# fmfi-compbio/nadavca

Hardware: NVIDIA B200
Metric: signal_samples_aligned_per_sec (higher is better)
Workload: dtype f64

## Files before the change

include/nadavca_b200.h:

```cpp
#ifndef NADAVCA_B200_H
#define NADAVCA_B200_H

#include <stdint.h>

#ifdef __cplusplus
extern "C" {
#endif

#define NVB_OK 0
#define NVB_EINVAL (-1)
#define NVB_ECUDA (-2)
#define NVB_ENOMEM (-3)
#define NVB_ESTATE (-4)

#define NVB_READ_OK 0
#define NVB_READ_NO_PATH 1
#define NVB_READ_BAD_BAND 2

typedef struct nvb_model nvb_model;
typedef struct nvb_batch nvb_batch;

int nvb_abi_version(void);
const char *nvb_last_error(void);
int nvb_device_count(void);
int nvb_trim_memory(int device);
#define NVB_SWEEP_AUTO 0
#define NVB_SWEEP_ROTATE 1
#define NVB_SWEEP_STRIPES 2
int nvb_set_sweep_schedule(int schedule);

nvb_model *nvb_model_create(int k, int central_position, int alphabet_size, const double *mean,
                            const double *sigma, int64_t n_kmers, int device);
void nvb_model_destroy(nvb_model *model);
int nvb_model_k(const nvb_model *model);
int nvb_model_central_position(const nvb_model *model);
int nvb_model_alphabet_size(const nvb_model *model);
int nvb_model_expected_signal(nvb_model *model, int32_t n_reads, const int32_t *reference,
                              const int64_t *reference_off, const int32_t *context_before,
                              const int64_t *context_before_off, const int32_t *context_after,
                              const int64_t *context_after_off, double *out);

typedef struct nvb_reads {
  int32_t n_reads;
  const double *signal;
  const int64_t *signal_off;
  const int32_t *reference;
  const int64_t *reference_off;
  const int32_t *context_before;
  const int64_t *context_before_off;
  const int32_t *context_after;
  const int64_t *context_after_off;
  const int32_t *anchors;
  const int64_t *anchor_off;
  int32_t bandwidth;
  int32_t min_event_length;
} nvb_reads;


int nvb_refine_alignment_batch(nvb_model *model, const nvb_reads *reads, int model_transitions, int32_t *events,
                               int32_t *status);
int nvb_estimate_log_likelihoods_batch(nvb_model *model, const nvb_reads *reads, int model_wobbling, double *out,
                                       int32_t *status);

nvb_batch *nvb_batch_create(nvb_model *model, const nvb_reads *reads);
void nvb_batch_destroy(nvb_batch *batch);
int nvb_batch_set_signal(nvb_batch *batch, const double *signal);
int nvb_batch_set_workspace_limit(nvb_batch *batch, int64_t bytes);
int nvb_batch_refine(nvb_batch *batch, int model_transitions, void *stream);
int nvb_batch_estimate(nvb_batch *batch, int model_wobbling, void *stream);
int nvb_batch_get_events(nvb_batch *batch, int32_t *events, int32_t *status);
int nvb_batch_get_log_likelihoods(nvb_batch *batch, double *out, int32_t *status);
int nvb_batch_get_bands(nvb_batch *batch, int32_t *starts, int32_t *ends);
int nvb_batch_cell_counts(nvb_batch *batch, int model_wobbling, int64_t counts[4]);
double *nvb_batch_d_log_likelihoods(nvb_batch *batch);
int32_t *nvb_batch_d_events(nvb_batch *batch);
int32_t *nvb_batch_d_status(nvb_batch *batch);
int nvb_batch_debug_rows(nvb_batch *batch, int read, int plane, double *out_log, int64_t n_cells);
int64_t nvb_batch_launch_count(const nvb_batch *batch);
#define NVB_N_STAGES 4
int nvb_batch_enable_timing(nvb_batch *batch, int on);
int nvb_batch_get_timing(nvb_batch *batch, double ms[NVB_N_STAGES], int64_t launches[NVB_N_STAGES]);
int nvb_measure_fp64_fma_rate(int device, double *fma_per_second);
// ... 50 lines not shown
```

nadavca_b200/_cabi.py:

```python
import ctypes
import os

import numpy as np

_HERE = os.path.dirname(os.path.abspath(__file__))
LIB_PATH = os.path.join(_HERE, 'libnadavca_b200.so')

NVB_READ_OK, NVB_READ_NO_PATH, NVB_READ_BAD_BAND = 0, 1, 2


class NadavcaCudaError(RuntimeError):
    pass


c_i32p = ctypes.POINTER(ctypes.c_int32)
c_i64p = ctypes.POINTER(ctypes.c_int64)
c_f64p = ctypes.POINTER(ctypes.c_double)
c_i8p = ctypes.POINTER(ctypes.c_int8)


class NvbReads(ctypes.Structure):
    _fields_ = [
        ('n_reads', ctypes.c_int32),
        ('signal', c_f64p), ('signal_off', c_i64p),
        ('reference', c_i32p), ('reference_off', c_i64p),
        ('context_before', c_i32p), ('context_before_off', c_i64p),
        ('context_after', c_i32p), ('context_after_off', c_i64p),
        ('anchors', c_i32p), ('anchor_off', c_i64p),
        ('bandwidth', ctypes.c_int32), ('min_event_length', ctypes.c_int32),
    ]


class NvbHits(ctypes.Structure):
    _fields_ = [
        ('n_reads', ctypes.c_int32),
        ('cigar_len', c_i32p), ('cigar_op', c_i8p), ('cigar_off', c_i64p),
        ('mapped_position', c_i64p), ('reverse', c_i32p),
        ('read_sequence', c_i8p), ('base_to_sample', c_i32p), ('read_off', c_i64p),
        ('n_signal', c_i32p),
        ('d_genome', ctypes.c_void_p), ('genome_length', ctypes.c_int64), ('bandwidth', ctypes.c_int32),
    ]


SIGNATURES = {
    'nvb_abi_version': (ctypes.c_int, []),
    'nvb_last_error': (ctypes.c_char_p, []),
    'nvb_device_count': (ctypes.c_int, []),
    'nvb_trim_memory': (ctypes.c_int, [ctypes.c_int]),
    'nvb_set_sweep_schedule': (ctypes.c_int, [ctypes.c_int]),
    'nvb_model_create': (ctypes.c_void_p, [ctypes.c_int, ctypes.c_int, ctypes.c_int, c_f64p, c_f64p, ctypes.c_int64,
                                           ctypes.c_int]),
    'nvb_model_destroy': (None, [ctypes.c_void_p]),
    'nvb_model_k': (ctypes.c_int, [ctypes.c_void_p]),
    'nvb_model_central_position': (ctypes.c_int, [ctypes.c_void_p]),
    'nvb_model_alphabet_size': (ctypes.c_int, [ctypes.c_void_p]),
    'nvb_model_expected_signal': (ctypes.c_int, [ctypes.c_void_p, ctypes.c_int32, c_i32p, c_i64p, c_i32p, c_i64p,
                                                 c_i32p, c_i64p, c_f64p]),
    'nvb_refine_alignment_batch': (ctypes.c_int, [ctypes.c_void_p, ctypes.POINTER(NvbReads), ctypes.c_int, c_i32p,
                                                  c_i32p]),
    'nvb_estimate_log_likelihoods_batch': (ctypes.c_int, [ctypes.c_void_p, ctypes.POINTER(NvbReads), ctypes.c_int,
                                                          c_f64p, c_i32p]),
    'nvb_batch_create': (ctypes.c_void_p, [ctypes.c_void_p, ctypes.POINTER(NvbReads)]),
    'nvb_batch_destroy': (None, [ctypes.c_void_p]),
    'nvb_batch_set_signal': (ctypes.c_int, [ctypes.c_void_p, c_f64p]),
    'nvb_batch_set_workspace_limit': (ctypes.c_int, [ctypes.c_void_p, ctypes.c_int64]),
    'nvb_batch_refine': (ctypes.c_int, [ctypes.c_void_p, ctypes.c_int, ctypes.c_void_p]),
    'nvb_batch_estimate': (ctypes.c_int, [ctypes.c_void_p, ctypes.c_int, ctypes.c_void_p]),
    'nvb_batch_get_events': (ctypes.c_int, [ctypes.c_void_p, c_i32p, c_i32p]),
    'nvb_batch_get_log_likelihoods': (ctypes.c_int, [ctypes.c_void_p, c_f64p, c_i32p]),
    'nvb_batch_get_bands': (ctypes.c_int, [ctypes.c_void_p, c_i32p, c_i32p]),
    'nvb_batch_cell_counts': (ctypes.c_int, [ctypes.c_void_p, ctypes.c_int, c_i64p]),
    'nvb_batch_d_log_likelihoods': (ctypes.c_void_p, [ctypes.c_void_p]),
    'nvb_batch_d_events': (ctypes.c_void_p, [ctypes.c_void_p]),
    'nvb_batch_d_status': (ctypes.c_void_p, [ctypes.c_void_p]),
    'nvb_batch_launch_count': (ctypes.c_int64, [ctypes.c_void_p]),
    'nvb_batch_debug_rows': (ctypes.c_int, [ctypes.c_void_p, ctypes.c_int, ctypes.c_int, c_f64p, ctypes.c_int64]),
    'nvb_batch_enable_timing': (ctypes.c_int, [ctypes.c_void_p, ctypes.c_int]),
    'nvb_batch_get_timing': (ctypes.c_int, [ctypes.c_void_p, c_f64p, c_i64p]),
    'nvb_measure_fp64_fma_rate': (ctypes.c_int, [ctypes.c_int, c_f64p]),
    'nvb_batch_get_alignment_table': (ctypes.c_int, [ctypes.c_void_p, c_i64p, c_i64p, c_i64p, c_i32p, c_i64p]),
    'nvb_batch_event_means': (ctypes.c_int, [ctypes.c_void_p, c_f64p]),
    'nvb_batch_apply_splines': (ctypes.c_int, [ctypes.c_void_p, c_f64p, c_f64p, c_i64p, ctypes.c_int, ctypes.c_void_p]),
    'nvb_batch_get_signal': (ctypes.c_int, [ctypes.c_void_p, c_f64p]),
    'nvb_batch_chunk_values': (ctypes.c_int, [ctypes.c_void_p, c_i32p, ctypes.c_double, ctypes.c_void_p,
                                              ctypes.c_void_p]),
    'nvb_batch_scatter_add': (ctypes.c_int, [ctypes.c_void_p, ctypes.c_void_p, c_i64p, ctypes.c_void_p,
                                             ctypes.c_void_p, ctypes.c_void_p]),
    'nvb_signal_anchors_batch': (ctypes.c_int, [ctypes.c_int, ctypes.POINTER(NvbHits), c_i32p, c_i64p,
                                                ctypes.c_void_p]),
    'nvb_radix_histogram_d': (ctypes.c_int, [ctypes.c_int, ctypes.c_void_p, ctypes.c_int64, ctypes.c_int,
                                             ctypes.c_double, ctypes.c_uint64, ctypes.c_int, ctypes.c_void_p,
                                             ctypes.c_void_p]),
    'nvb_normalize_each': (ctypes.c_int, [ctypes.c_int, c_f64p, c_i64p, ctypes.c_int32, ctypes.c_double,
                                          ctypes.c_double, c_f64p, c_f64p, ctypes.c_void_p]),
    'nvb_normalize_clip_d': (ctypes.c_int, [ctypes.c_int, ctypes.c_void_p, ctypes.c_int64, ctypes.c_double,
                                            ctypes.c_double, ctypes.c_double, ctypes.c_double, ctypes.c_void_p,
                                            ctypes.c_void_p]),
    'nvb_batch_scatter_add_rows': (ctypes.c_int, [ctypes.c_void_p, ctypes.c_void_p, c_i64p, ctypes.c_void_p,
                                                  ctypes.c_void_p]),
    'nvb_posterior_rows_d': (ctypes.c_int, [ctypes.c_int, ctypes.c_void_p, ctypes.c_int64, ctypes.c_int64,
                                            ctypes.c_int64, ctypes.c_void_p, ctypes.c_void_p, ctypes.c_int32,
                                            ctypes.c_int, ctypes.c_double, ctypes.c_void_p, ctypes.c_void_p]),
# ... 117 lines not shown
```

nadavca_b200/csrc/api.cu:

```cuda
#include <math.h>
#include <stdarg.h>
#include <stdio.h>
#include <stdlib.h>
#include <string.h>

#include <algorithm>
#include <map>
#include <mutex>
#include <string>
#include <vector>

#include "../../include/nadavca_b200.h"
#include "kernels.h"

namespace {

thread_local std::string g_err;
thread_local int g_code = 0;

struct Options {
  int sweep = NVB_SWEEP_AUTO;
  bool skip_path = false;
  int sweep_warps = 0;
  Options() {
    if (const char *env = getenv("NVB_SWEEP")) sweep = env[0] == 'r' ? NVB_SWEEP_ROTATE : (env[0] == 's' ? NVB_SWEEP_STRIPES : NVB_SWEEP_AUTO);
    skip_path = getenv("NVB_DEBUG_SKIP_PATH") != nullptr;
    if (const char *env = getenv("NVB_SWEEP_WARPS")) sweep_warps = atoi(env);
  }
};
Options g_opt;

int fail(int code, const char *fmt, ...) {
  char buf[512];
  va_list ap;
  va_start(ap, fmt);
  vsnprintf(buf, sizeof buf, fmt, ap);
  va_end(ap);
  g_err = buf;
  g_code = code;
  return code;
}

#define CU(expr)                                                                                      \
  do {                                                                                                \
    cudaError_t _e = (expr);                                                                          \
    if (_e != cudaSuccess)                                                                            \
      return fail(NVB_ECUDA, "CUDA error %s at %s:%d (%s)", cudaGetErrorString(_e), __FILE__, __LINE__, #expr); \
  } while (0)

struct DevicePool {
  std::mutex m;
  std::multimap<size_t, void *> free_blocks;
  size_t cached = 0;
};
DevicePool g_pool[64];

void pool_trim(int device) {
  DevicePool &P = g_pool[device & 63];
  std::lock_guard<std::mutex> lock(P.m);
  for (auto &kv : P.free_blocks) cudaFree(kv.second);
  P.free_blocks.clear();
  P.cached = 0;
}

cudaError_t pool_alloc(void **out, size_t bytes, size_t *capacity, int *device) {
  bytes = (std::max<size_t>(bytes, 1) + 511) & ~(size_t)511;
  int dev = 0;
  cudaError_t e = cudaGetDevice(&dev);
  if (e != cudaSuccess) return e;
  *device = dev;
  DevicePool &P = g_pool[dev & 63];
  {
    std::lock_guard<std::mutex> lock(P.m);
    auto it = P.free_blocks.lower_bound(bytes);
    if (it != P.free_blocks.end() && it->first <= bytes + bytes / 4 + (1 << 20)) {
      *out = it->second; *capacity = it->first;
      P.cached -= it->first;
      P.free_blocks.erase(it);
      return cudaSuccess;
    }
// ... 98 lines not shown
  std::vector<int32_t> h_rev;
  std::vector<int64_t> h_dest;
  DevBuf<int64_t> d_mat_base, d_dp_base, d_rec_base;
  int64_t ws_limit = 0;
  int64_t launches = 0;
  int path_pk = 11;
  cudaStream_t run_stream = nullptr;
  std::vector<cudaStream_t> streams_used;
  Workspace *last_ws = nullptr;
  void touch(cudaStream_t st) {
    run_stream = st;
    if (std::find(streams_used.begin(), streams_used.end(), st) == streams_used.end()) streams_used.push_back(st);
  }
  void drain() {
    for (cudaStream_t st : streams_used) cudaStreamSynchronize(st);
  }
  int plan_mode = -1;
  bool plan_dp = false;
  int64_t plan_limit = -1;
  int64_t plan_max[3] = {0, 0, 0};
  std::vector<Wave> plan_waves_cache;
  BatchDev dev{};
  bool timing = false;
  std::vector<std::pair<int, std::pair<cudaEvent_t, cudaEvent_t>>> timed;
  ~nvb_batch() {
    for (auto &t : timed) { cudaEventDestroy(t.second.first); cudaEventDestroy(t.second.second); }
  }
};

namespace {
struct StageTimer {
  nvb_batch *b; cudaStream_t st; cudaEvent_t e0 = nullptr, e1 = nullptr; int stage;
  StageTimer(nvb_batch *batch, int stage_, cudaStream_t stream) : b(batch), st(stream), stage(stage_) {
    if (b->timing) { cudaEventCreate(&e0); cudaEventCreate(&e1); cudaEventRecord(e0, st); }
  }
  ~StageTimer() {
    if (b->timing) { cudaEventRecord(e1, st); b->timed.push_back({stage, {e0, e1}}); }
  }
};
}

extern "C" {

int nvb_abi_version(void) { return 1; }

const char *nvb_last_error(void) { return g_err.c_str(); }

int nvb_set_sweep_schedule(int schedule) {
  const int before = g_opt.sweep;
  if (schedule == NVB_SWEEP_AUTO || schedule == NVB_SWEEP_ROTATE || schedule == NVB_SWEEP_STRIPES) g_opt.sweep = schedule;
  return before;
}

int nvb_device_count(void) {
  int n = 0;
  if (cudaGetDeviceCount(&n) != cudaSuccess) { cudaGetLastError(); return 0; }
  return n;
}

nvb_model *nvb_model_create(int k, int central_position, int alphabet_size, const double *mean,
                            const double *sigma, int64_t n_kmers, int device) {
  if (k <= 0 || alphabet_size < 2 || central_position < 0 || central_position >= k || !mean || !sigma) {
    fail(NVB_EINVAL, "nvb_model_create: bad arguments");
    return nullptr;
  }
  int64_t expect = 1;
  for (int i = 0; i < k; i++) expect *= alphabet_size;
  if (n_kmers != expect) {
    fail(NVB_EINVAL, "nvb_model_create: expected %lld k-mers, got %lld", (long long)expect, (long long)n_kmers);
    return nullptr;
  }
  if (nvb_device_count() <= device || device < 0) {
    fail(NVB_ECUDA, "nvb_model_create: CUDA device %d not available (no CPU fallback)", device);
    return nullptr;
  }
  if (cudaSetDevice(device) != cudaSuccess) { fail(NVB_ECUDA, "cudaSetDevice(%d) failed", device); return nullptr; }
  nvb_model *m = new nvb_model();
  m->device = device;
  {
    int sms = 0;
    if (cudaDeviceGetAttribute(&sms, cudaDevAttrMultiProcessorCount, device) == cudaSuccess && sms > 0) m->sm_count = sms;
  }
  std::vector<double> ac(n_kmers), mc(n_kmers);
  for (int64_t i = 0; i < n_kmers; i++) {
    double s = sigma[i];
    ac[i] = log(1 / sqrt(2 * M_PI * s * s));
    mc[i] = 1 / (2 * s * s);
  }
  if (upload(m->mean, mean, (size_t)n_kmers, 0) != cudaSuccess || upload(m->ac, ac.data(), (size_t)n_kmers, 0) != cudaSuccess ||
      upload(m->mc, mc.data(), (size_t)n_kmers, 0) != cudaSuccess || cudaStreamSynchronize(0) != cudaSuccess) {
    fail(NVB_ECUDA, "nvb_model_create: upload failed: %s", cudaGetErrorString(cudaGetLastError()));
    delete m;
    return nullptr;
  }
  m->dev.k = k; m->dev.central = central_position; m->dev.alphabet = alphabet_size; m->dev.n_kmers = n_kmers;
  m->dev.mean = m->mean.p; m->dev.ac = m->ac.p; m->dev.mc = m->mc.p;
  m->dev.log_p_in = log(0.01);
  return m;
}

void nvb_model_destroy(nvb_model *model) {
  if (!model) return;
  const int device = model->device;
  cudaSetDevice(device);
  cudaDeviceSynchronize();
  delete model;
// ... 281 lines not shown
  for (const Wave &w : waves) {
    {
      StageTimer t(b, 0, st);
      const int src = run_sweep(b, ws, mode, w, st);
      if (src == -1) return fail(NVB_EINVAL, "min_event_length %d is not supported (maximum 6)", b->dev.mel);
      if (src) return fail(NVB_ENOMEM, "cannot allocate the hand-off rows of the sweep for a band row of %d columns", w.maxw);
    }
    if (!g_opt.skip_path) {
      StageTimer t(b, 1, st);
      nvbk_score(w.cells, ws.pF.p, ws.pX.p, ws.sF.p, ws.sX.p, st);
      if (nvbk_path2(b->dev, mode, w.b0, w.b1, b->path_pk, b->d_mat_base.p, ws.pF.p, ws.records.p, b->d_rec_base.p,
                     ws.dp.p, b->d_dp_base.p, w.maxw, b->d_events.p, b->d_status.p, st))
        return fail(NVB_ECUDA, "path kernel: cannot reserve shared memory");
    }
    b->launches += 1;
    b->launches += 2;
  }
  CU(cudaGetLastError());
  b->have_events = true;
  return NVB_OK;
}

int nvb_batch_estimate(nvb_batch *b, int model_wobbling, void *stream) {
  if (!b) return fail(NVB_EINVAL, "NULL batch");
  CU(cudaSetDevice(b->model->device));
  cudaStream_t st = (cudaStream_t)stream;
  const ModelDev &M = b->model->dev;
  const int mode = model_wobbling ? NVB_MODE_WOBBLE : NVB_MODE_PLAIN;
  if (M.k + 2 > 32) return fail(NVB_EINVAL, "k = %d is too large for the SNP kernel (needs k+2 <= 32 lanes)", M.k);
  std::vector<Wave> waves;
  Workspace &ws = b->model->workspace(st);
  b->touch(st);
  b->last_ws = &ws;
  int rc = prepare_workspace(b, ws, mode, false, waves, st);
  if (rc) return rc;
  CU(b->d_ll.alloc((size_t)b->total_ref * M.alphabet, st, true));
  nvbk_fill_status(b->dev, b->d_status.p, b->d_ll.p, M.alphabet, st);
  b->launches++;
  for (const Wave &w : waves) {
    {
      StageTimer t(b, 0, st);
      const int src = run_sweep(b, ws, mode, w, st);
      if (src == -1) return fail(NVB_EINVAL, "min_event_length %d is not supported (maximum 6)", b->dev.mel);
      if (src) return fail(NVB_ENOMEM, "cannot allocate the hand-off rows of the sweep for a band row of %d columns", w.maxw);
    }
    {
      StageTimer t(b, 2, st);
      nvbk_no_snp2(M, b->dev, w.b0, w.b1, b->d_mat_base.p, ws.pF.p, ws.pX.p, ws.sF.p, ws.sX.p, b->d_ll.p, st);
    }
    int snp_rc;
    {
      StageTimer t(b, 3, st);
      snp_rc = nvbk_snp2(M, b->dev, model_wobbling, w.b0, w.b1, b->ref_off[w.b0], b->ref_off[w.b1],
                         b->d_mat_base.p, ws.pF.p, ws.pX.p, ws.sF.p, ws.sX.p, b->d_ll.p, st);
    }
    if (snp_rc) return fail(NVB_EINVAL, "SNP kernel configuration not supported");
    b->launches += 3;
  }
  CU(cudaGetLastError());
  b->have_ll = true;
  return NVB_OK;
}

int nvb_batch_get_events(nvb_batch *b, int32_t *events, int32_t *status) {
  if (!b) return fail(NVB_EINVAL, "NULL batch");
  if (!b->have_events) return fail(NVB_ESTATE, "nvb_batch_get_events before nvb_batch_refine");
  CU(cudaSetDevice(b->model->device));
  cudaStream_t st = b->run_stream;
  if (events) CU(cudaMemcpyAsync(events, b->d_events.p, (size_t)2 * b->total_ref * sizeof(int32_t), cudaMemcpyDeviceToHost, st));
  if (status) CU(cudaMemcpyAsync(status, b->d_status.p, (size_t)b->n_reads * sizeof(int32_t), cudaMemcpyDeviceToHost, st));
  CU(cudaStreamSynchronize(st));
  return NVB_OK;
}

int nvb_batch_get_log_likelihoods(nvb_batch *b, double *out, int32_t *status) {
  if (!b) return fail(NVB_EINVAL, "NULL batch");
  if (!b->have_ll) return fail(NVB_ESTATE, "nvb_batch_get_log_likelihoods before nvb_batch_estimate");
  CU(cudaSetDevice(b->model->device));
  cudaStream_t st = b->run_stream;
  if (out) CU(cudaMemcpyAsync(out, b->d_ll.p, (size_t)b->total_ref * b->model->dev.alphabet * sizeof(double), cudaMemcpyDeviceToHost, st));
  if (status) CU(cudaMemcpyAsync(status, b->d_status.p, (size_t)b->n_reads * sizeof(int32_t), cudaMemcpyDeviceToHost, st));
  CU(cudaStreamSynchronize(st));
  return NVB_OK;
}

int nvb_batch_get_bands(nvb_batch *b, int32_t *starts, int32_t *ends) {
  if (!b) return fail(NVB_EINVAL, "NULL batch");
  CU(cudaSetDevice(b->model->device));
  size_t cnt = (size_t)b->total_ref + b->n_reads;
  if (starts) CU(cudaMemcpy(starts, b->d_bs.p, cnt * sizeof(int32_t), cudaMemcpyDeviceToHost));
  if (ends) CU(cudaMemcpy(ends, b->d_be.p, cnt * sizeof(int32_t), cudaMemcpyDeviceToHost));
  return NVB_OK;
}

int nvb_batch_cell_counts(nvb_batch *b, int model_wobbling, int64_t counts[4]) {
  if (!b || !counts) return fail(NVB_EINVAL, "NULL argument");
  CU(cudaSetDevice(b->model->device));
  size_t cnt = (size_t)b->total_ref + b->n_reads;
  std::vector<int32_t> bs(cnt), be(cnt);
  CU(cudaMemcpy(bs.data(), b->d_bs.p, cnt * sizeof(int32_t), cudaMemcpyDeviceToHost));
  CU(cudaMemcpy(be.data(), b->d_be.p, cnt * sizeof(int32_t), cudaMemcpyDeviceToHost));
  const int k = b->model->dev.k, cp = b->model->dev.central, A = b->model->dev.alphabet;
  int64_t c0 = 0, c1 = 0, c2 = 0, c3 = 0;
  for (int r = 0; r < b->n_reads; r++) {
    if (b->flags[r]) continue;
    const int n = (int)(b->ref_off[r + 1] - b->ref_off[r]);
    const int32_t *s = bs.data() + b->ref_off[r] + r, *e = be.data() + b->ref_off[r] + r;
// ... 392 lines not shown
```

nadavca_b200/csrc/kernels.h:

```cpp
#pragma once
#include "common.cuh"

void nvbk_band(const BatchDev &B, int64_t *d_summary, cudaStream_t st);
void nvbk_row_emission(const ModelDev &M, const BatchDev &B, int64_t total, double scale, double *d_out, cudaStream_t st);
double nvbk_emission_scale();
void nvbk_expected_signal(const ModelDev &M, const BatchDev &B, int64_t total, double *d_out, cudaStream_t st);

int64_t nvbk_sweep2_global_handoff_doubles(int mode, int n_reads, int wave_maxw, int force_warps);
int nvbk_sweep2(const ModelDev &M, const BatchDev &B, int mode, int b0, int b1, int wave_maxw, int force_warps,
                const int64_t *d_mat_base, double *pF, int32_t *pX, double *sF, int32_t *sX, double *g_handoff,
                cudaStream_t st);
int nvbk_sweep_rotate(const ModelDev &M, const BatchDev &B, int mode, int b0, int b1, const int64_t *d_mat_base,
                      double *pF, int32_t *pX, double *sF, int32_t *sX, cudaStream_t st);
void nvbk_no_snp2(const ModelDev &M, const BatchDev &B, int b0, int b1, const int64_t *d_mat_base, const double *pF,
                  const int32_t *pX, const double *sF, const int32_t *sX, double *d_out_ll, cudaStream_t st);

int nvbk_snp2(const ModelDev &M, const BatchDev &B, int wobbling, int b0, int b1, int64_t g0, int64_t g1,
              const int64_t *d_mat_base, const double *pF, const int32_t *pX, const double *sF, const int32_t *sX,
              double *d_out_ll, cudaStream_t st);

int nvbk_path2_columns_per_lane(int maxw);
void nvbk_score(int64_t total_cells, double *pF, const int32_t *pX, const double *sF, const int32_t *sX,
                cudaStream_t st);
int nvbk_path2(const BatchDev &B, int mode, int b0, int b1, int pk, const int64_t *d_mat_base, const double *score,
               uint32_t *d_records, const int64_t *d_rec_base, double *d_dp, const int64_t *d_dp_base, int wave_maxw,
               int32_t *d_events, int32_t *d_status, cudaStream_t st);

void nvbk_alignment_table(const BatchDev &B, const int32_t *d_events, const int32_t *d_status,
                          const int64_t *d_sig_start, const int64_t *d_ref_start, const int64_t *d_ref_end,
                          const int32_t *d_reverse, int64_t total, int64_t *d_out, cudaStream_t st);
void nvbk_event_means(const BatchDev &B, const int32_t *d_events, const int32_t *d_status, int64_t total, double *d_out,
                      cudaStream_t st);
void nvbk_apply_splines(const BatchDev &B, double *d_signal, const double *d_knots, const double *d_coefs,
                        const int64_t *d_spl_off, int degree, int64_t total, cudaStream_t st);
void nvbk_chunk_values(const BatchDev &B, const double *d_ll, const int32_t *d_reverse, double nel, int64_t total,
                       double *d_chunks, cudaStream_t st);
void nvbk_scatter_add(const BatchDev &B, const double *d_chunks, const int64_t *d_dest, const int32_t *d_status,
                      int64_t total, double *d_acc, int32_t *d_cov, cudaStream_t st);
void nvbk_posterior(const double *d_ll, const int8_t *d_ref, const int64_t *d_group_off, int n_groups,
                    int64_t total, int k, double snp_prior, double *d_out, cudaStream_t st);
void nvbk_scatter_add_rows(const BatchDev &B, const double *d_chunks, const int64_t *d_dest, const int32_t *d_status,
                           int64_t total, double *d_rows, cudaStream_t st);
void nvbk_posterior_rows(const double *d_rows, int64_t base, int64_t row_lo, int64_t row_hi, const int8_t *d_ref,
                         const int64_t *d_group_off, int n_groups, int k, double snp_prior, double *d_out,
                         cudaStream_t st);
void nvbk_fill_status(const BatchDev &B, int32_t *d_status, double *d_ll, int alphabet, cudaStream_t st);

void nvbk_radix_hist(const double *d_values, int64_t n, int mode, double shift, unsigned long long prefix, int fixed,
                     unsigned long long *d_hist, cudaStream_t st);
void nvbk_normalize_each(const double *d_values, const int64_t *d_off, int n_reads, double lo, double hi, double *d_out,
                         double *d_shift_scale, cudaStream_t st);
void nvbk_normalize_clip(const double *d_values, int64_t n, double shift, double scale, double lo, double hi,
                         double *d_out, cudaStream_t st);

void nvbk_anchors(const AnchorBatch &A, int32_t *d_anchors, int64_t *d_meta, cudaStream_t st);

float nvbk_fp64_fma_probe(int iters, int blocks, cudaStream_t st, double *d_sink);
```

nadavca_b200/csrc/snp3.cu:

```cuda
#include "dp3.cuh"
#include "kernels.h"

namespace {

#ifndef NVB_SNP_RENORM_MASK
#define NVB_SNP_RENORM_MASK 15
#endif

template <int MEL, int MODE>
__global__ void __launch_bounds__(128) snp3_kernel(ModelDev M, BatchDev B, int b0, int b1, int64_t g0, int64_t n_tasks,
                                                   int LT, int TPW, const int64_t *mat_base, const double *pF,
                                                   const int32_t *pX, const double *sF, const int32_t *sX,
                                                   double *out_ll) {
  constexpr bool wobbling = (MODE == NVB_MODE_WOBBLE);
  const unsigned exp_tab = exp_table_init();
  const int wic = threadIdx.x >> 5, lane = threadIdx.x & 31;
  const int64_t warp_id = blockIdx.x * (int64_t)(blockDim.x >> 5) + wic;
  const int A = M.alphabet;
  const double C_E2 = 0.1353352832366127;

  const int slot = lane / LT, ri = lane - slot * LT;
  const int64_t task = warp_id * TPW + slot;
  const bool have = slot < TPW && task < n_tasks;

  LaneCfg L;
  lane_cfg_clear(L);
  const double *rowF = nullptr;
  const int32_t *rowX = nullptr;
  const double *sig = B.signal;
  int N = 1, C0 = 0, T = 0;
  double *out = nullptr;

  if (have) {
    const int64_t g = g0 + task / (A - 1);
    const int alt = (int)(task % (A - 1));
    int lo = b0, hi = b1;
    while (hi - lo > 1) {
      const int mid = (lo + hi) >> 1;
      if (B.ref_off[mid] <= g) lo = mid; else hi = mid;
    }
    const int b = lo;
    if (!B.flags[b]) {
      ReadView v = read_view(B, b);
      const int n = v.n;
      const int i = (int)(g - B.ref_off[b]);
      const int refbase = v.ref[i];
      const int base = alt + (alt >= refbase ? 1 : 0);
      const int back = M.k - M.central - 1, fwd = M.central;
      const int first = max(0, i - back), last = min(n - 1, i + fwd);
      const int npairs = last - first + 1;
      N = v.N; sig = v.sig;
      C0 = v.bs[first];
      const int64_t mb = mat_base[b];
      int kmer_at = -1;
      bool hasA = false;
      if (ri == 0) {
        L.role = NVB_ROLE_LOADER;
        L.ms = v.bs[first]; L.me = v.be[first];
        rowF = pF + mb + v.coff[first]; rowX = pX + mb + v.coff[first];
        kmer_at = first > 0 ? first - 1 : first;
      } else if (ri <= npairs) {
        const int j = first + ri - 1;
        L.role = NVB_ROLE_PAIR;
        hasA = wobbling && j > 0;
        if (hasA) { L.ws = v.bs[j]; L.we = v.be[j]; }
        L.ms = v.bs[j + 1]; L.me = v.be[j + 1];
        kmer_at = j;
      } else if (ri == npairs + 1) {
        L.role = NVB_ROLE_JOIN;
        hasA = wobbling && last + 1 < n;
        if (hasA) { L.ws = v.bs[last]; L.we = v.be[last]; }
        L.ms = v.bs[last + 1]; L.me = v.be[last + 1];
        rowF = sF + mb + v.coff[last + 1]; rowX = sX + mb + v.coff[last + 1];
        kmer_at = last + 1 < n ? last + 1 : last;
        out = out_ll + (B.ref_off[b] + i) * A + base;
        const int endcol = hasA ? L.we : L.me;
        T = endcol - C0 + ri + 1 + MEL;
      }
      if (hasA) { L.cm = C_E2; L.abias = 0; }
      if (kmer_at >= 0) {
        const int id = kmer_id(M, v, kmer_at, i, base);
        lane_set_emission(L, M.mean[id], M.ac[id], M.mc[id]);
      }
    }
  }
  T = __reduce_max_sync(NVB_FULL, T);

  LaneState<MEL> S;
  lane_reset(S);
  LaneOut res;
  res.f = 0.0; res.E = NVB_EZERO; res.p = 1.0; res.k = 0;
  const bool is_loader = L.role == NVB_ROLE_LOADER, is_join = L.role == NVB_ROLE_JOIN;
  const bool reads_row = is_loader || is_join;
  const bool passes = L.role == NVB_ROLE_PAIR;
  for (int t0 = 0; t0 < T; t0 += NVB_SNP_RENORM_MASK + 1) {
    const int t1 = min(t0 + NVB_SNP_RENORM_MASK + 1, T);
#pragma unroll 1
    for (int t = t0; t < t1; t++) {
      const int c = C0 + (t - ri);
      const double x = __ldg(sig + min(max(c - 1, 0), N - 1));
      LaneOut in = shfl_up_out<MODE>(res);
      double rF = 0.0;
      int rX = NVB_EZERO;
      if (reads_row && c >= L.ms && c <= L.me) {
        rF = __ldg(rowF + (c - L.ms));
        rX = __ldg(rowX + (c - L.ms));
      }
      XD aout;
      lane_step<MEL, MODE, true, false>(L, S, exp_tab, c, x, in, is_join ? rF : 1.0, is_join ? rX : 0, res, aout);
      if (is_loader) {
        res.f = rF; res.E = rX;
      } else if (!passes) {
        res.f = 0.0; res.E = NVB_EZERO;
      }
    }
    lane_renorm(S);
  }
  if (is_join) {
    xd_renorm(S.mod);
    *out = log_ext(S.mod.f, S.mod.e);
  }
}

template <int MEL>
void launch_snp3(const ModelDev &M, const BatchDev &B, int wobbling, int b0, int b1, int64_t g0, int64_t n_tasks, int LT,
                 int TPW, const int64_t *mb, const double *pF, const int32_t *pX, const double *sF, const int32_t *sX,
                 double *out, cudaStream_t st) {
  const int warps = 4;
  const int64_t n_warps = (n_tasks + TPW - 1) / TPW;
  const unsigned grid = (unsigned)((n_warps + warps - 1) / warps);
  if (wobbling)
    snp3_kernel<MEL, NVB_MODE_WOBBLE><<<grid, warps * NVB_WARP, 0, st>>>(M, B, b0, b1, g0, n_tasks, LT, TPW, mb, pF, pX,
                                                                         sF, sX, out);
  else
    snp3_kernel<MEL, NVB_MODE_PLAIN><<<grid, warps * NVB_WARP, 0, st>>>(M, B, b0, b1, g0, n_tasks, LT, TPW, mb, pF, pX,
                                                                        sF, sX, out);
}

}

int nvbk_snp2(const ModelDev &M, const BatchDev &B, int wobbling, int b0, int b1, int64_t g0, int64_t g1,
              const int64_t *d_mat_base, const double *pF, const int32_t *pX, const double *sF, const int32_t *sX,
              double *d_out_ll, cudaStream_t st) {
  const int LT = M.k + 2;
  if (LT > NVB_WARP) return -1;
  const int TPW = NVB_WARP / LT;
  const int64_t n_tasks = (g1 - g0) * (M.alphabet - 1);
  if (n_tasks <= 0) return 0;
#define NVB_SNP3(MEL) \
  launch_snp3<MEL>(M, B, wobbling, b0, b1, g0, n_tasks, LT, TPW, d_mat_base, pF, pX, sF, sX, d_out_ll, st)
  switch (B.mel) {
    case 0: NVB_SNP3(0); break;
    case 1: NVB_SNP3(1); break;
    case 2: NVB_SNP3(2); break;
    case 3: NVB_SNP3(3); break;
    case 4: NVB_SNP3(4); break;
    case 5: NVB_SNP3(5); break;
    case 6: NVB_SNP3(6); break;
    default: return -1;
  }
#undef NVB_SNP3
  return 0;
}
```

nadavca_b200/dtw.py:

```python
import ctypes

import numpy as np

from . import _cabi
from ._cabi import NadavcaCudaError, ReadsPack


class KmerModel:

    def __init__(self, k, central_position, alphabet_size, mean, sigma, device=None):
        self._k = int(k)
        self._central_position = int(central_position)
        self._alphabet_size = int(alphabet_size)
        self.mean = np.ascontiguousarray(mean, dtype=np.float64)
        self.sigma = np.ascontiguousarray(sigma, dtype=np.float64)
        if self.mean.shape != self.sigma.shape or self.mean.size != self._alphabet_size ** self._k:
            raise ValueError('mean and sigma need alphabet_size**k entries')
        self._device = device
        self._handle = None

    def get_k(self):
        return self._k

    def get_central_position(self):
# ... 196 lines not shown
        return [out[off[i]:off[i + 1]] for i in range(self.n_reads)]

    def chunk_values(self, reverse, normalization_event_length, d_chunks, stream=None):
        r = _cabi.as_array(reverse, np.int32)
        _cabi.check(self.lib.nvb_batch_chunk_values(self.handle, _cabi.ptr(r, ctypes.c_int32),
                                                    float(normalization_event_length), ctypes.c_void_p(d_chunks),
                                                    _stream(stream)), 'nvb_batch_chunk_values')

    def scatter_add(self, d_chunks, dest, d_acc, d_cov, stream=None):
        d = _cabi.as_array(dest, np.int64)
        _cabi.check(self.lib.nvb_batch_scatter_add(self.handle, ctypes.c_void_p(d_chunks),
                                                   _cabi.ptr(d, ctypes.c_int64), ctypes.c_void_p(d_acc),
                                                   ctypes.c_void_p(d_cov), _stream(stream)), 'nvb_batch_scatter_add')

    def scatter_add_rows(self, d_chunks, dest, d_rows, stream=None):
        d = _cabi.as_array(dest, np.int64)
        _cabi.check(self.lib.nvb_batch_scatter_add_rows(self.handle, ctypes.c_void_p(d_chunks),
                                                        _cabi.ptr(d, ctypes.c_int64), ctypes.c_void_p(d_rows),
                                                        _stream(stream)), 'nvb_batch_scatter_add_rows')

    def debug_rows(self, read, plane, transitions=False):
        bs, be = self.bands()[read]
        w = be - bs + 1
        cells = int(2 * w.sum() - w[0] - w[-1]) if transitions else int(w.sum())
        out = np.zeros(cells, dtype=np.float64)
        _cabi.check(self.lib.nvb_batch_debug_rows(self.handle, int(read), int(plane),
                                                  _cabi.ptr(out, ctypes.c_double), cells), 'nvb_batch_debug_rows')
        return out

    @property
    def launch_count(self):
        return int(self.lib.nvb_batch_launch_count(self.handle))

    STAGES = ('rows', 'path', 'no_snp', 'snp')

    def enable_timing(self, on=True):
        _cabi.check(self.lib.nvb_batch_enable_timing(self.handle, int(on)), 'nvb_batch_enable_timing')

    def timing(self):
        ms = np.zeros(4, dtype=np.float64)
        cnt = np.zeros(4, dtype=np.int64)
        _cabi.check(self.lib.nvb_batch_get_timing(self.handle, _cabi.ptr(ms, ctypes.c_double),
                                                  _cabi.ptr(cnt, ctypes.c_int64)), 'nvb_batch_get_timing')
        return {name: (float(ms[i]), int(cnt[i])) for i, name in enumerate(self.STAGES)}


SWEEP_SCHEDULES = {None: 0, 'auto': 0, 'r': 1, 'rotate': 1, 's': 2, 'stripes': 2}


def set_sweep_schedule(schedule):
    return int(_cabi.load().nvb_set_sweep_schedule(SWEEP_SCHEDULES[schedule]))


def trim_memory(device=None):
    from .read import trim_staging
    lib = _cabi.require_device()
    _cabi.check(lib.nvb_trim_memory(_current_device() if device is None else int(device)), 'nvb_trim_memory')
    trim_staging()


def measure_fp64_fma_rate(device=0):
    lib = _cabi.require_device()
    out = ctypes.c_double(0)
    _cabi.check(lib.nvb_measure_fp64_fma_rate(int(device), ctypes.byref(out)), 'nvb_measure_fp64_fma_rate')
    return out.value


def _stream(stream):
    if stream is None:
        return ctypes.c_void_p(0)
    return ctypes.c_void_p(int(getattr(stream, 'cuda_stream', stream)))


def posterior(device, d_ll, d_ref, group_off, k, snp_prior, d_out, stream=None):
    lib = _cabi.require_device()
    g = _cabi.as_array(group_off, np.int64)
    _cabi.check(lib.nvb_posterior(int(device), ctypes.c_void_p(d_ll), ctypes.c_void_p(d_ref),
                                  _cabi.ptr(g, ctypes.c_int64), len(g) - 1, int(k), float(snp_prior),
                                  ctypes.c_void_p(d_out), _stream(stream)), 'nvb_posterior')


def posterior_resident(device, d_ll, d_ref, d_group_off, n_groups, total, k, snp_prior, d_out, stream=None):
    lib = _cabi.require_device()
    _cabi.check(lib.nvb_posterior_d(int(device), ctypes.c_void_p(d_ll), ctypes.c_void_p(d_ref),
                                    ctypes.c_void_p(d_group_off), int(n_groups), int(total), int(k), float(snp_prior),
                                    ctypes.c_void_p(d_out), _stream(stream)), 'nvb_posterior_d')


def posterior_rows(device, d_rows, base_row, row_lo, row_hi, d_ref, d_group_off, n_groups, k, snp_prior, d_out_rows,
                   stream=None):
    lib = _cabi.require_device()
    _cabi.check(lib.nvb_posterior_rows_d(int(device), ctypes.c_void_p(d_rows), int(base_row), int(row_lo), int(row_hi),
                                         ctypes.c_void_p(d_ref), ctypes.c_void_p(d_group_off), int(n_groups), int(k),
                                         float(snp_prior), ctypes.c_void_p(d_out_rows), _stream(stream)),
                'nvb_posterior_rows_d')



def refine_alignment(signal, reference, context_before, context_after, approximate_alignment, bandwidth,
                     min_event_length, kmer_model, model_transitions):
    with Batch(kmer_model, [signal], [reference], [context_before], [context_after], [approximate_alignment],
               bandwidth, min_event_length) as batch:
        batch.refine(model_transitions)
        events, _ = batch.events()
    return [] if events[0] is None else events[0].tolist()

# ... 9 lines not shown
```

Baseline: 202.2 million.

## Map two SNP DP rows per lane to pack more tasks per warp

The SNP kernel can now give each lane R=2 consecutive DP rows instead of one. A skewed in-register wavefront steps between the two rows, so each warp holds roughly twice as many SNP tasks. The default layout picks R=2 whenever k+2 is even, and an environment variable or API call can force the old one-row layout. The intent is to cut idle lanes and warp count in the SNP stage. In exchange each lane does twice the serial work and holds more registers, and a leaner path is specialised for warps where no join row falls in the first slot.

```diff
diff --git a/include/nadavca_b200.h b/include/nadavca_b200.h
--- a/include/nadavca_b200.h
+++ b/include/nadavca_b200.h
@@ -28,6 +28,8 @@
 #define NVB_SWEEP_ROTATE 1
 #define NVB_SWEEP_STRIPES 2
 int nvb_set_sweep_schedule(int schedule);
+int nvb_set_snp_layout(int rows_per_lane);
+int nvb_snp_rows_per_lane(int k, int layout);
 
 nvb_model *nvb_model_create(int k, int central_position, int alphabet_size, const double *mean,
                             const double *sigma, int64_t n_kmers, int device);
diff --git a/nadavca_b200/_cabi.py b/nadavca_b200/_cabi.py
--- a/nadavca_b200/_cabi.py
+++ b/nadavca_b200/_cabi.py
@@ -48,6 +48,8 @@
     'nvb_device_count': (ctypes.c_int, []),
     'nvb_trim_memory': (ctypes.c_int, [ctypes.c_int]),
     'nvb_set_sweep_schedule': (ctypes.c_int, [ctypes.c_int]),
+    'nvb_set_snp_layout': (ctypes.c_int, [ctypes.c_int]),
+    'nvb_snp_rows_per_lane': (ctypes.c_int, [ctypes.c_int, ctypes.c_int]),
     'nvb_model_create': (ctypes.c_void_p, [ctypes.c_int, ctypes.c_int, ctypes.c_int, c_f64p, c_f64p, ctypes.c_int64,
                                            ctypes.c_int]),
     'nvb_model_destroy': (None, [ctypes.c_void_p]),
diff --git a/nadavca_b200/csrc/api.cu b/nadavca_b200/csrc/api.cu
--- a/nadavca_b200/csrc/api.cu
+++ b/nadavca_b200/csrc/api.cu
@@ -22,10 +22,15 @@
   int sweep = NVB_SWEEP_AUTO;
   bool skip_path = false;
   int sweep_warps = 0;
+  int snp_layout = 0;
   Options() {
     if (const char *env = getenv("NVB_SWEEP")) sweep = env[0] == 'r' ? NVB_SWEEP_ROTATE : (env[0] == 's' ? NVB_SWEEP_STRIPES : NVB_SWEEP_AUTO);
     skip_path = getenv("NVB_DEBUG_SKIP_PATH") != nullptr;
     if (const char *env = getenv("NVB_SWEEP_WARPS")) sweep_warps = atoi(env);
+    if (const char *env = getenv("NVB_SNP_LAYOUT")) {
+      const int r = atoi(env);
+      if (r == 1 || r == 2) snp_layout = r;
+    }
   }
 };
 Options g_opt;
@@ -230,6 +235,19 @@
   return before;
 }
 
+int nvb_set_snp_layout(int rows_per_lane) {
+  const int before = g_opt.snp_layout;
+  if (rows_per_lane >= 0 && rows_per_lane <= 2) g_opt.snp_layout = rows_per_lane;
+  return before;
+}
+
+int nvb_snp_rows_per_lane(int k, int layout) {
+  if (k < 1 || k + 2 > NVB_WARP) return NVB_EINVAL;
+  if (layout < 0) layout = g_opt.snp_layout;
+  if (layout > 2) return NVB_EINVAL;
+  return nvbk_snp_rows_per_lane(k, layout);
+}
+
 int nvb_device_count(void) {
   int n = 0;
   if (cudaGetDeviceCount(&n) != cudaSuccess) { cudaGetLastError(); return 0; }
@@ -617,7 +635,7 @@
     {
       StageTimer t(b, 3, st);
       snp_rc = nvbk_snp2(M, b->dev, model_wobbling, w.b0, w.b1, b->ref_off[w.b0], b->ref_off[w.b1],
-                         b->d_mat_base.p, ws.pF.p, ws.pX.p, ws.sF.p, ws.sX.p, b->d_ll.p, st);
+                         b->d_mat_base.p, ws.pF.p, ws.pX.p, ws.sF.p, ws.sX.p, b->d_ll.p, g_opt.snp_layout, st);
     }
     if (snp_rc) return fail(NVB_EINVAL, "SNP kernel configuration not supported");
     b->launches += 3;
diff --git a/nadavca_b200/csrc/kernels.h b/nadavca_b200/csrc/kernels.h
--- a/nadavca_b200/csrc/kernels.h
+++ b/nadavca_b200/csrc/kernels.h
@@ -17,7 +17,8 @@
 
 int nvbk_snp2(const ModelDev &M, const BatchDev &B, int wobbling, int b0, int b1, int64_t g0, int64_t g1,
               const int64_t *d_mat_base, const double *pF, const int32_t *pX, const double *sF, const int32_t *sX,
-              double *d_out_ll, cudaStream_t st);
+              double *d_out_ll, int layout, cudaStream_t st);
+int nvbk_snp_rows_per_lane(int k, int layout);
 
 int nvbk_path2_columns_per_lane(int maxw);
 void nvbk_score(int64_t total_cells, double *pF, const int32_t *pX, const double *sF, const int32_t *sX,
diff --git a/nadavca_b200/csrc/snp3.cu b/nadavca_b200/csrc/snp3.cu
--- a/nadavca_b200/csrc/snp3.cu
+++ b/nadavca_b200/csrc/snp3.cu
@@ -7,87 +7,80 @@
 #define NVB_SNP_RENORM_MASK 15
 #endif
 
+struct SnpTask {
+  ReadView v;
+  int i, base, first, last, npairs;
+  int64_t mb;
+  double *out;
+};
+
+__device__ __forceinline__ bool snp_task(const ModelDev &M, const BatchDev &B, int b0, int b1, int64_t g0, int64_t task,
+                                         const int64_t *mat_base, double *out_ll, SnpTask &K) {
+  const int A = M.alphabet;
+  const int64_t g = g0 + task / (A - 1);
+  const int alt = (int)(task % (A - 1));
+  int lo = b0, hi = b1;
+  while (hi - lo > 1) {
+    const int mid = (lo + hi) >> 1;
+    if (B.ref_off[mid] <= g) lo = mid; else hi = mid;
+  }
+  const int b = lo;
+  if (B.flags[b]) return false;
+  K.v = read_view(B, b);
+  K.i = (int)(g - B.ref_off[b]);
+  const int refbase = K.v.ref[K.i];
+  K.base = alt + (alt >= refbase ? 1 : 0);
+  const int back = M.k - M.central - 1, fwd = M.central;
+  K.first = max(0, K.i - back);
+  K.last = min(K.v.n - 1, K.i + fwd);
+  K.npairs = K.last - K.first + 1;
+  K.mb = mat_base[b];
+  K.out = out_ll + (B.ref_off[b] + K.i) * A + K.base;
+  return true;
+}
+
+template <int MEL, bool wobbling>
+__device__ __forceinline__ void snp_row(const ModelDev &M, const SnpTask &K, int ri, const double *pF,
+                                        const int32_t *pX, const double *sF, const int32_t *sX, LaneCfg &L,
+                                        const double *&rowF, const int32_t *&rowX, int &T) {
+  const double C_E2 = 0.1353352832366127;
+  const ReadView &v = K.v;
+  const int n = v.n, first = K.first, last = K.last, npairs = K.npairs;
+  const int C0 = v.bs[first];
+  int kmer_at = -1;
+  bool hasA = false;
+  if (ri == 0) {
+    L.role = NVB_ROLE_LOADER;
+    L.ms = v.bs[first]; L.me = v.be[first];
+    rowF = pF + K.mb + v.coff[first]; rowX = pX + K.mb + v.coff[first];
+    kmer_at = first > 0 ? first - 1 : first;
+  } else if (ri <= npairs) {
+    const int j = first + ri - 1;
+    L.role = NVB_ROLE_PAIR;
+    hasA = wobbling && j > 0;
+    if (hasA) { L.ws = v.bs[j]; L.we = v.be[j]; }
+    L.ms = v.bs[j + 1]; L.me = v.be[j + 1];
+    kmer_at = j;
+  } else if (ri == npairs + 1) {
+    L.role = NVB_ROLE_JOIN;
+    hasA = wobbling && last + 1 < n;
+    if (hasA) { L.ws = v.bs[last]; L.we = v.be[last]; }
+    L.ms = v.bs[last + 1]; L.me = v.be[last + 1];
+    rowF = sF + K.mb + v.coff[last + 1]; rowX = sX + K.mb + v.coff[last + 1];
+    kmer_at = last + 1 < n ? last + 1 : last;
+    const int endcol = hasA ? L.we : L.me;
+    T = endcol - C0 + ri + 1 + MEL;
+  }
+  if (hasA) { L.cm = C_E2; L.abias = 0; }
+  if (kmer_at >= 0) {
+    const int id = kmer_id(M, v, kmer_at, K.i, K.base);
+    lane_set_emission(L, M.mean[id], M.ac[id], M.mc[id]);
+  }
+}
+
 template <int MEL, int MODE>
-__global__ void __launch_bounds__(128) snp3_kernel(ModelDev M, BatchDev B, int b0, int b1, int64_t g0, int64_t n_tasks,
-                                                   int LT, int TPW, const int64_t *mat_base, const double *pF,
-                                                   const int32_t *pX, const double *sF, const int32_t *sX,
-                                                   double *out_ll) {
-  constexpr bool wobbling = (MODE == NVB_MODE_WOBBLE);
-  const unsigned exp_tab = exp_table_init();
-  const int wic = threadIdx.x >> 5, lane = threadIdx.x & 31;
-  const int64_t warp_id = blockIdx.x * (int64_t)(blockDim.x >> 5) + wic;
-  const int A = M.alphabet;
-  const double C_E2 = 0.1353352832366127;
-
-  const int slot = lane / LT, ri = lane - slot * LT;
-  const int64_t task = warp_id * TPW + slot;
-  const bool have = slot < TPW && task < n_tasks;
-
-  LaneCfg L;
-  lane_cfg_clear(L);
-  const double *rowF = nullptr;
-  const int32_t *rowX = nullptr;
-  const double *sig = B.signal;
-  int N = 1, C0 = 0, T = 0;
-  double *out = nullptr;
-
-  if (have) {
-    const int64_t g = g0 + task / (A - 1);
-    const int alt = (int)(task % (A - 1));
-    int lo = b0, hi = b1;
-    while (hi - lo > 1) {
-      const int mid = (lo + hi) >> 1;
-      if (B.ref_off[mid] <= g) lo = mid; else hi = mid;
-    }
-    const int b = lo;
-    if (!B.flags[b]) {
-      ReadView v = read_view(B, b);
-      const int n = v.n;
-      const int i = (int)(g - B.ref_off[b]);
-      const int refbase = v.ref[i];
-      const int base = alt + (alt >= refbase ? 1 : 0);
-      const int back = M.k - M.central - 1, fwd = M.central;
-      const int first = max(0, i - back), last = min(n - 1, i + fwd);
-      const int npairs = last - first + 1;
-      N = v.N; sig = v.sig;
-      C0 = v.bs[first];
-      const int64_t mb = mat_base[b];
-      int kmer_at = -1;
-      bool hasA = false;
-      if (ri == 0) {
-        L.role = NVB_ROLE_LOADER;
-        L.ms = v.bs[first]; L.me = v.be[first];
-        rowF = pF + mb + v.coff[first]; rowX = pX + mb + v.coff[first];
-        kmer_at = first > 0 ? first - 1 : first;
-      } else if (ri <= npairs) {
-        const int j = first + ri - 1;
-        L.role = NVB_ROLE_PAIR;
-        hasA = wobbling && j > 0;
-        if (hasA) { L.ws = v.bs[j]; L.we = v.be[j]; }
-        L.ms = v.bs[j + 1]; L.me = v.be[j + 1];
-        kmer_at = j;
-      } else if (ri == npairs + 1) {
-        L.role = NVB_ROLE_JOIN;
-        hasA = wobbling && last + 1 < n;
-        if (hasA) { L.ws = v.bs[last]; L.we = v.be[last]; }
-        L.ms = v.bs[last + 1]; L.me = v.be[last + 1];
-        rowF = sF + mb + v.coff[last + 1]; rowX = sX + mb + v.coff[last + 1];
-        kmer_at = last + 1 < n ? last + 1 : last;
-        out = out_ll + (B.ref_off[b] + i) * A + base;
-        const int endcol = hasA ? L.we : L.me;
-        T = endcol - C0 + ri + 1 + MEL;
-      }
-      if (hasA) { L.cm = C_E2; L.abias = 0; }
-      if (kmer_at >= 0) {
-        const int id = kmer_id(M, v, kmer_at, i, base);
-        lane_set_emission(L, M.mean[id], M.ac[id], M.mc[id]);
-      }
-    }
-  }
-  T = __reduce_max_sync(NVB_FULL, T);
-
-  LaneState<MEL> S;
-  lane_reset(S);
+__device__ __forceinline__ void snp_steps1(const LaneCfg &L, const double *rowF, const int32_t *rowX, unsigned exp_tab,
+                                           const double *sig, int N, int C0, int ri, int T, LaneState<MEL> &S) {
   LaneOut res;
   res.f = 0.0; res.E = NVB_EZERO; res.p = 1.0; res.k = 0;
   const bool is_loader = L.role == NVB_ROLE_LOADER, is_join = L.role == NVB_ROLE_JOIN;
@@ -108,21 +101,127 @@
       }
       XD aout;
       lane_step<MEL, MODE, true, false>(L, S, exp_tab, c, x, in, is_join ? rF : 1.0, is_join ? rX : 0, res, aout);
-      if (is_loader) {
-        res.f = rF; res.E = rX;
-      } else if (!passes) {
-        res.f = 0.0; res.E = NVB_EZERO;
+      res.f = is_loader ? rF : (passes ? res.f : 0.0);
+      res.E = is_loader ? rX : (passes ? res.E : NVB_EZERO);
+    }
+    lane_renorm(S);
+  }
+}
+
+template <int MEL, int MODE, bool CAN_LOAD, bool CAN_JOIN>
+__device__ __forceinline__ void slot_step(const LaneCfg &L, LaneState<MEL> &S, unsigned exp_tab, int c, double x,
+                                          const LaneOut &in, const double *rowF, const int32_t *rowX, LaneOut &res) {
+  const bool is_loader = CAN_LOAD && L.role == NVB_ROLE_LOADER;
+  const bool is_join = CAN_JOIN && L.role == NVB_ROLE_JOIN;
+  double rF = 0.0;
+  int rX = NVB_EZERO;
+  if ((is_loader || is_join) && c >= L.ms && c <= L.me) {
+    rF = __ldg(rowF + (c - L.ms));
+    rX = __ldg(rowX + (c - L.ms));
+  }
+  XD aout;
+  lane_step<MEL, MODE, CAN_JOIN, false>(L, S, exp_tab, c, x, in, is_join ? rF : 1.0, is_join ? rX : 0, res, aout);
+  res.f = is_loader ? rF : res.f;
+  res.E = is_loader ? rX : res.E;
+}
+
+template <int MEL, int MODE, int R, bool JOIN_ANY, int s>
+__device__ __forceinline__ void slots_down(const LaneCfg (&L)[R], LaneState<MEL> (&S)[R], LaneOut (&res)[R],
+                                           const double *const (&rowF)[R], const int32_t *const (&rowX)[R],
+                                           unsigned exp_tab, int c, const double (&xb)[R], int u, const LaneOut &in0) {
+  slot_step<MEL, MODE, s == 0, JOIN_ANY || s == R - 1>(L[s], S[s], exp_tab, c - s, xb[(u - s + R) % R],
+                                                       s == 0 ? in0 : res[s > 0 ? s - 1 : 0], rowF[s], rowX[s], res[s]);
+  if constexpr (s > 0) slots_down<MEL, MODE, R, JOIN_ANY, s - 1>(L, S, res, rowF, rowX, exp_tab, c, xb, u, in0);
+}
+
+template <int MEL, int MODE, int R, bool JOIN_ANY>
+__device__ __forceinline__ void snp_steps(const LaneCfg (&L)[R], const double *const (&rowF)[R],
+                                          const int32_t *const (&rowX)[R], unsigned exp_tab, const double *sig, int N,
+                                          int cb, int T, LaneState<MEL> (&S)[R]) {
+  LaneOut res[R];
+  double xb[R];
+#pragma unroll
+  for (int s = 0; s < R; s++) { res[s].f = 0.0; res[s].E = NVB_EZERO; res[s].p = 1.0; res[s].k = 0; }
+#pragma unroll
+  for (int d = 1; d < R; d++) xb[R - d] = __ldg(sig + min(max(cb - d - 1, 0), N - 1));
+  for (int t0 = 0; t0 < T; t0 += NVB_SNP_RENORM_MASK + 1) {
+    const int t1 = min(t0 + NVB_SNP_RENORM_MASK + 1, T);
+#pragma unroll 1
+    for (int t = t0; t < t1; t += R) {
+#pragma unroll
+      for (int u = 0; u < R; u++) {
+        const int c = cb + t + u;
+        xb[u] = __ldg(sig + min(max(c - 1, 0), N - 1));
+        const LaneOut in0 = shfl_up_out<MODE>(res[R - 1]);
+        slots_down<MEL, MODE, R, JOIN_ANY, R - 1>(L, S, res, rowF, rowX, exp_tab, c, xb, u, in0);
       }
     }
-    lane_renorm(S);
-  }
-  if (is_join) {
-    xd_renorm(S.mod);
-    *out = log_ext(S.mod.f, S.mod.e);
-  }
-}
-
-template <int MEL>
+#pragma unroll
+    for (int s = 0; s < R; s++) lane_renorm(S[s]);
+  }
+}
+
+template <int MEL, int MODE, int R>
+__global__ void __launch_bounds__(128) snp3_kernel(ModelDev M, BatchDev B, int b0, int b1, int64_t g0, int64_t n_tasks,
+                                                   int LT, int TPW, const int64_t *mat_base, const double *pF,
+                                                   const int32_t *pX, const double *sF, const int32_t *sX,
+                                                   double *out_ll) {
+  constexpr bool wobbling = (MODE == NVB_MODE_WOBBLE);
+  const unsigned exp_tab = exp_table_init();
+  const int wic = threadIdx.x >> 5, lane = threadIdx.x & 31;
+  const int64_t warp_id = blockIdx.x * (int64_t)(blockDim.x >> 5) + wic;
+
+  const int LPT = LT / R;
+  const int tiw = lane / LPT, lr = lane - tiw * LPT;
+  const int64_t task = warp_id * TPW + tiw;
+  const bool have = tiw < TPW && task < n_tasks;
+
+  LaneCfg L[R];
+  const double *rowF[R];
+  const int32_t *rowX[R];
+#pragma unroll
+  for (int s = 0; s < R; s++) { lane_cfg_clear(L[s]); rowF[s] = nullptr; rowX[s] = nullptr; }
+  const double *sig = B.signal;
+  int N = 1, C0 = 0, T = 0;
+  double *out = nullptr;
+
+  if (have) {
+    SnpTask K;
+    if (snp_task(M, B, b0, b1, g0, task, mat_base, out_ll, K)) {
+      N = K.v.N; sig = K.v.sig;
+      C0 = K.v.bs[K.first];
+      out = K.out;
+#pragma unroll
+      for (int s = 0; s < R; s++) snp_row<MEL, wobbling>(M, K, lr * R + s, pF, pX, sF, sX, L[s], rowF[s], rowX[s], T);
+    }
+  }
+  T = __reduce_max_sync(NVB_FULL, T);
+
+  LaneState<MEL> S[R];
+#pragma unroll
+  for (int s = 0; s < R; s++) lane_reset(S[s]);
+  if constexpr (R == 1) {
+    snp_steps1<MEL, MODE>(L[0], rowF[0], rowX[0], exp_tab, sig, N, C0, lr, T, S[0]);
+  } else {
+    T = (T + R - 1) / R * R;
+    bool lean = true;
+#pragma unroll
+    for (int s = 0; s < R - 1; s++) lean = lean && L[s].role != NVB_ROLE_JOIN;
+    if (__all_sync(NVB_FULL, lean))
+      snp_steps<MEL, MODE, R, false>(L, rowF, rowX, exp_tab, sig, N, C0 - lr * R, T, S);
+    else
+      snp_steps<MEL, MODE, R, true>(L, rowF, rowX, exp_tab, sig, N, C0 - lr * R, T, S);
+  }
+#pragma unroll
+  for (int s = 0; s < R; s++) {
+    if (L[s].role == NVB_ROLE_JOIN) {
+      xd_renorm(S[s].mod);
+      *out = log_ext(S[s].mod.f, S[s].mod.e);
+    }
+  }
+}
+
+template <int MEL, int R>
 void launch_snp3(const ModelDev &M, const BatchDev &B, int wobbling, int b0, int b1, int64_t g0, int64_t n_tasks, int LT,
                  int TPW, const int64_t *mb, const double *pF, const int32_t *pX, const double *sF, const int32_t *sX,
                  double *out, cudaStream_t st) {
@@ -130,25 +229,18 @@
   const int64_t n_warps = (n_tasks + TPW - 1) / TPW;
   const unsigned grid = (unsigned)((n_warps + warps - 1) / warps);
   if (wobbling)
-    snp3_kernel<MEL, NVB_MODE_WOBBLE><<<grid, warps * NVB_WARP, 0, st>>>(M, B, b0, b1, g0, n_tasks, LT, TPW, mb, pF, pX,
-                                                                         sF, sX, out);
+    snp3_kernel<MEL, NVB_MODE_WOBBLE, R><<<grid, warps * NVB_WARP, 0, st>>>(M, B, b0, b1, g0, n_tasks, LT, TPW, mb, pF,
+                                                                            pX, sF, sX, out);
   else
-    snp3_kernel<MEL, NVB_MODE_PLAIN><<<grid, warps * NVB_WARP, 0, st>>>(M, B, b0, b1, g0, n_tasks, LT, TPW, mb, pF, pX,
-                                                                        sF, sX, out);
-}
-
-}
-
-int nvbk_snp2(const ModelDev &M, const BatchDev &B, int wobbling, int b0, int b1, int64_t g0, int64_t g1,
-              const int64_t *d_mat_base, const double *pF, const int32_t *pX, const double *sF, const int32_t *sX,
-              double *d_out_ll, cudaStream_t st) {
-  const int LT = M.k + 2;
-  if (LT > NVB_WARP) return -1;
-  const int TPW = NVB_WARP / LT;
-  const int64_t n_tasks = (g1 - g0) * (M.alphabet - 1);
-  if (n_tasks <= 0) return 0;
-#define NVB_SNP3(MEL) \
-  launch_snp3<MEL>(M, B, wobbling, b0, b1, g0, n_tasks, LT, TPW, d_mat_base, pF, pX, sF, sX, d_out_ll, st)
+    snp3_kernel<MEL, NVB_MODE_PLAIN, R><<<grid, warps * NVB_WARP, 0, st>>>(M, B, b0, b1, g0, n_tasks, LT, TPW, mb, pF,
+                                                                           pX, sF, sX, out);
+}
+
+template <int R>
+void launch_snp3_mel(const ModelDev &M, const BatchDev &B, int wobbling, int b0, int b1, int64_t g0, int64_t n_tasks,
+                     int LT, int TPW, const int64_t *mb, const double *pF, const int32_t *pX, const double *sF,
+                     const int32_t *sX, double *out, cudaStream_t st) {
+#define NVB_SNP3(MEL) launch_snp3<MEL, R>(M, B, wobbling, b0, b1, g0, n_tasks, LT, TPW, mb, pF, pX, sF, sX, out, st)
   switch (B.mel) {
     case 0: NVB_SNP3(0); break;
     case 1: NVB_SNP3(1); break;
@@ -157,8 +249,32 @@
     case 4: NVB_SNP3(4); break;
     case 5: NVB_SNP3(5); break;
     case 6: NVB_SNP3(6); break;
-    default: return -1;
   }
 #undef NVB_SNP3
+}
+
+}
+
+int nvbk_snp_rows_per_lane(int k, int layout) {
+  const int LT = k + 2;
+  const int R = layout > 0 ? (LT % layout == 0 ? layout : 1) : (LT % 2 == 0 ? 2 : 1);
+  return R;
+}
+
+int nvbk_snp2(const ModelDev &M, const BatchDev &B, int wobbling, int b0, int b1, int64_t g0, int64_t g1,
+              const int64_t *d_mat_base, const double *pF, const int32_t *pX, const double *sF, const int32_t *sX,
+              double *d_out_ll, int layout, cudaStream_t st) {
+  const int LT = M.k + 2;
+  if (LT > NVB_WARP) return -1;
+  const int TPW = NVB_WARP / LT;
+  const int64_t n_tasks = (g1 - g0) * (M.alphabet - 1);
+  if (n_tasks <= 0) return 0;
+  if (B.mel < 0 || B.mel > 6) return -1;
+  const int R = nvbk_snp_rows_per_lane(M.k, layout);
+  const int TPW_R = NVB_WARP / (LT / R);
+  if (R == 2)
+    launch_snp3_mel<2>(M, B, wobbling, b0, b1, g0, n_tasks, LT, TPW_R, d_mat_base, pF, pX, sF, sX, d_out_ll, st);
+  else
+    launch_snp3_mel<1>(M, B, wobbling, b0, b1, g0, n_tasks, LT, TPW, d_mat_base, pF, pX, sF, sX, d_out_ll, st);
   return 0;
 }
diff --git a/nadavca_b200/dtw.py b/nadavca_b200/dtw.py
--- a/nadavca_b200/dtw.py
+++ b/nadavca_b200/dtw.py
@@ -272,6 +272,19 @@
     return int(_cabi.load().nvb_set_sweep_schedule(SWEEP_SCHEDULES[schedule]))
 
 
+def set_snp_layout(rows_per_lane):
+    r = 0 if rows_per_lane is None else int(rows_per_lane)
+    if r not in (0, 1, 2):
+        raise ValueError('SNP layout must be None, 0, 1 or 2, not %r' % (rows_per_lane,))
+    return int(_cabi.load().nvb_set_snp_layout(r))
+
+
+def snp_rows_per_lane(k, layout=None):
+    r = int(_cabi.load().nvb_snp_rows_per_lane(int(k), -1 if layout is None else int(layout)))
+    _cabi.check(min(r, 0), 'nvb_snp_rows_per_lane')
+    return r
+
+
 def trim_memory(device=None):
     from .read import trim_staging
     lib = _cabi.require_device()
```

Result: faster. 210.8 million, median of 6 (+4.3%).
